# huzjkevin/planar_optical_flow

Measured on AMD Instinct MI355X. Metric: scans/sec, flow-only preprocess of 450-pt synthetic scan pairs, batch 4096 per GPU (+ flow EPE vs reference oracle), higher is better.
Workload: dtype f32 flow arithmetic (float32 outputs) + f64 exact association / mask decisions; the float64-output instantiation (the reference's float64 operation order) is `value_f64`

## Files before the change

planar_optical_flow_amd/csrc/scan_flow.hip:

```cpp
#include <cmath>
#include <cstdlib>
#include <type_traits>

#include "pof_common.h"

namespace {

constexpr int kThreads = 256;

__global__ void laser_phi_kernel(double start, double stop, double step, int n, double *tab)
{
    int i = blockIdx.x * blockDim.x + threadIdx.x;
    if (i >= n) return;
    double p = (double)i * step;
    p = p + start;
    if (i == n - 1 && n > 1) p = stop;
    double s, c;
    sincos(p, &s, &c);
    tab[i] = p;
    tab[n + 2 * i] = c;
    tab[n + 2 * i + 1] = s;
}

struct PreArgs {
// ... 542 lines not shown
                    gx[k] = gy[k] = 0.0f;
                    if (bidx[k] > 0) {
                        double wx, wy;
                        if (ndet[q] <= kInline) {
                            wx = s_det[q][bidx[k] - 1][0];
                            wy = s_det[q][bidx[k] - 1][1];
                            cls[k] = s_lab[q][bidx[k] - 1];
                        } else {
                            const double *w = a.ws_det + (long long)(dfirst + bidx[k] - 1) * kDetStride;
                            wx = w[0];
                            wy = w[1];
                            cls[k] = (long long)w[4];
                        }
                        gx[k] = (float)(wy * cs[k] - wx * sn[k]);
                        gy[k] = (float)((wx * cs[k] + wy * sn[k]) - (double)r[q][k]);
                    }
                }
                if (PTS == 2) {
                    if (a.closest) stream_ll2(reinterpret_cast<long long *>(a.closest), o / 2, bidx[0], bidx[PTS - 1]);
                    if (a.target_cls) stream_ll2(reinterpret_cast<long long *>(a.target_cls), o / 2, cls[0], cls[PTS - 1]);
                    if (a.target_reg) stream_f4(a.target_reg, o / 2, gx[0], gy[0], gx[PTS - 1], gy[PTS - 1]);
                } else {
                    if (a.closest) a.closest[o] = bidx[0];
                    if (a.target_cls) a.target_cls[o] = cls[0];
                    if (a.target_reg) reinterpret_cast<float2 *>(a.target_reg)[o] = make_float2(gx[0], gy[0]);
                }
            }
        }

        if (ok) {
            if (PTS == 2) {
                if (a.dyn_mask) stream_f2(a.dyn_mask, o / 2, dmask[0], dmask[PTS - 1]);
                if (a.valid_mask) stream_f2(a.valid_mask, o / 2, vmask[0], vmask[PTS - 1]);
                if (a.exclude_mask) stream_f2(a.exclude_mask, o / 2, dmask[0] * vmask[0], dmask[PTS - 1] * vmask[PTS - 1]);
            } else {
                if (a.dyn_mask) a.dyn_mask[o] = dmask[0];
                if (a.valid_mask) a.valid_mask[o] = vmask[0];
                if (a.exclude_mask) a.exclude_mask[o] = dmask[0] * vmask[0];
            }
        }
    }
}

constexpr int kMaxSlots = POF_SCAN_MAX_SLOTS;
constexpr int kWaveLds = 2 * kImgBytes;

enum : unsigned {
    kOutXy = 1u << 0, kOutFlow = 1u << 1, kHasDets = 1u << 2, kOutClosest = 1u << 3, kOutCls = 1u << 4,
    kOutReg = 1u << 5, kOutDyn = 1u << 6, kOutValid = 1u << 7, kOutExcl = 1u << 8, kCanonical = 1u << 9,
    kKindShift = 10,
};
constexpr int kCfgHeadline = (int)(kOutFlow | kHasDets | kOutCls | kOutReg | kOutExcl | kCanonical);

struct FlatBatch {
    const float *ranges;
    long long sample_stride;
    void *xy, *flow;
    int64_t *closest, *target_cls;
    float *target_reg, *dyn_mask, *valid_mask, *exclude_mask;
    const int32_t *det_offsets;
    const double *ws_rec, *ws_det;
    int B;
    int wave0;
};
static_assert(sizeof(FlatBatch) % 8 == 0, "FlatBatch is read from the kernel arguments in 8-byte words");

struct FlatArgs {
    const double *tab;
    const float *tabf;
    int N, halfN;
    unsigned magic_m;
    int magic_s;
    unsigned flags;
    int nb;
    int total_waves;
    int main_blocks;
    double ra[3], sd[3], sa[3];
    int lb[3];
    float m_dyn;
    float thr_assoc;
    float m_assoc;
    int uni_waves;
    unsigned uni_m;
    int uni_s;
    int pad_[2];
    int wave0[kMaxSlots];
    FlatBatch b[kMaxSlots];
};

struct ParamsMulti {
    int nb;
    int first, total;
    int uni_blocks;
    unsigned uni_m;
    int uni_s;
    int blk0[kMaxSlots + 1];
    PreArgs p[kMaxSlots];
};

template <typename T>
__device__ __forceinline__ T fma_t(T a, T b, T c);
template <>
__device__ __forceinline__ double fma_t<double>(double a, double b, double c) { return fma(a, b, c); }
template <>
__device__ __forceinline__ float fma_t<float>(float a, float b, float c) { return fmaf(a, b, c); }

template <typename T>
__device__ __forceinline__ void apply_motion_t(int kind, T px, T py, T m0, T m1, T m2, T m3, T t0, T t1, T dph,
                                               T &fx, T &fy)
{
    if (kind == 0) {
        fx = fma_t<T>(py, m1, px * m0) - t0;
        fy = fma_t<T>(py, m3, px * m2) - t1;
    } else if (kind == 1) {
        fx = (fma_t<T>(py, m1, px * m0) - t0) - px;
        fy = (fma_t<T>(py, m3, px * m2) - t1) - py;
    } else if (kind == 2) {
        fx = -t0 - (py * -dph);
        fy = -t1 - (px * dph);
    } else if (kind == 3) {
        fx = ((T)0 - m0 * py + m1) * m3;
        fy = ((m0 * px - (T)0) + m2) * m3;
    } else {
        fx = fma_t<T>(py, m1, px * m0) + t0;
        fy = fma_t<T>(py, m3, px * m2) + t1;
    }
}

template <int CFG>
struct FlatCfg {
    unsigned rt;
    __device__ __forceinline__ bool has(unsigned bit) const { return CFG >= 0 ? ((unsigned)CFG & bit) != 0 : (rt & bit) != 0; }
    __device__ __forceinline__ int kind() const { return CFG >= 0 ? (CFG >> kKindShift) & 7 : (int)(rt >> kKindShift) & 7; }
};

using D2V = double __attribute__((ext_vector_type(2)));

struct RunLoads {
    float2 rv;
    float4 tf;
    D2V t0v, t1v;
    int local, q;
    bool ok;
};

template <typename OutT>
__device__ __forceinline__ RunLoads flat_loads(const FlatArgs &L, const FlatBatch &bt, const int lane, const int sA,
                                               const int l0)
{
    constexpr bool kF32 = sizeof(OutT) == 4;
    RunLoads in;
    int local = l0 + lane;
    const int q = local >= L.halfN ? 1 : 0;
    local -= q ? L.halfN : 0;
    in.local = local;
    in.q = q;
    in.ok = sA + q < bt.B;
    const unsigned i0 = 2u * (unsigned)local;
    const GLOBAL_AS float *rowA = (const GLOBAL_AS float *)bt.ranges + (long long)sA * bt.sample_stride;
    const unsigned roff = (q && in.ok ? (unsigned)bt.sample_stride : 0u) + i0;
    const F2V rr = *(const GLOBAL_AS F2V *)(rowA + roff);
    in.rv = make_float2(rr.x, rr.y);
    in.tf = make_float4(0.f, 0.f, 0.f, 0.f);
    in.t0v = D2V{0.0, 0.0};
    in.t1v = D2V{0.0, 0.0};
    if (kF32 && L.tabf) {
        in.tf = *reinterpret_cast<const float4 *>(L.tabf + 2u * i0);
    } else {
        const double *tab_cs = L.tab + L.N;
        in.t0v = *reinterpret_cast<const D2V *>(tab_cs + 2u * i0);
        in.t1v = *reinterpret_cast<const D2V *>(tab_cs + 2u * i0 + 2);
    }
    return in;
}

template <typename OutT, int CFG>
__device__ __forceinline__ void flat_run(const FlatArgs &L, const FlatBatch &bt, const FlatCfg<CFG> cfg,
                                         const unsigned char *lds, const int lane, const int sA, const int l0,
                                         const long long pair0, const RunLoads &in)
{
    constexpr bool kF32 = sizeof(OutT) == 4;
    const int halfN = L.halfN, N = L.N;
    const int local = in.local, q = in.q;
    const int b = sA + q;
    const bool ok = in.ok;
    const int i0 = 2 * local;
    const float2 rv = in.rv;
    const double *tab_cs = L.tab + N;
    float csf[2], snf[2];
    const D2V t0v = in.t0v, t1v = in.t1v;
    if (kF32 && L.tabf) {
        csf[0] = in.tf.x; snf[0] = in.tf.y; csf[1] = in.tf.z; snf[1] = in.tf.w;
    } else {
        csf[0] = (float)t0v.x; snf[0] = (float)t0v.y; csf[1] = (float)t1v.x; snf[1] = (float)t1v.y;
    }
    const float r[2] = {rv.x, rv.y};
    F2V pxf = {r[0] * csf[0], r[1] * csf[1]}, pyf = {r[0] * snf[0], r[1] * snf[1]};
    auto cs64 = [&](int k) { return tab_cs[2u * (unsigned)(i0 + k)]; };
    auto sn64 = [&](int k) { return tab_cs[2u * (unsigned)(i0 + k) + 1]; };
    auto p64x = [&](int k) { return (double)r[k] * cs64(k); };
    auto p64y = [&](int k) { return (double)r[k] * sn64(k); };
    const unsigned char *hdr = lds + q * kImgBytes;

    if (cfg.has(kOutXy) && ok) {
        OutT *xy = static_cast<OutT *>(bt.xy) + 4 * pair0;
        store2<OutT>(xy, 2u * (unsigned)lane, p64x(0), p64y(0));
        store2<OutT>(xy, 2u * (unsigned)lane + 1, p64x(1), p64y(1));
    }

    if (cfg.has(kOutFlow)) {
        const int kind = cfg.kind();
        if (kF32 && kind != 1) {
            const float4 ma = *reinterpret_cast<const float4 *>(hdr);
            const float4 mb = *reinterpret_cast<const float4 *>(hdr + 16);
            float fxs[2], fys[2];
#pragma unroll
            for (int k = 0; k < 2; ++k) {
                float fx, fy;
                apply_motion_t<float>(kind, pxf[k], pyf[k], ma.x, ma.y, ma.z, ma.w, mb.x, mb.y, mb.z, fx, fy);
                if (cfg.has(kCanonical)) {
                    const float gx = fmaf(csf[k], fx, -snf[k] * fy);
                    const float gy = fmaf(snf[k], fx, csf[k] * fy);
                    fx = gx;
                    fy = gy;
                }
                fxs[k] = fx;
                fys[k] = fy;
            }
            if (ok) stream_f4(reinterpret_cast<float *>(bt.flow) + 4 * pair0, (unsigned)lane, fxs[0], fys[0], fxs[1], fys[1]);
        } else {
            const double *mot = reinterpret_cast<const double *>(hdr + kImgMot);
            const double m0 = mot[0], m1 = mot[1], m2 = mot[2], m3 = mot[3];
            const double tr0 = mot[4], tr1 = mot[5], dph = mot[6];
            OutT *fl = static_cast<OutT *>(bt.flow) + 4 * pair0;
            double cs[2], sn[2];
            if (kF32 && L.tabf) {
                cs[0] = cs64(0); sn[0] = sn64(0); cs[1] = cs64(1); sn[1] = sn64(1);
            } else {
                cs[0] = t0v.x; sn[0] = t0v.y; cs[1] = t1v.x; sn[1] = t1v.y;
            }
            double f[4];
#pragma unroll
            for (int k = 0; k < 2; ++k) {
                double fx, fy;
                apply_motion(kind, (double)r[k] * cs[k], (double)r[k] * sn[k], m0, m1, m2, m3, tr0, tr1, dph, fx, fy);
                if (cfg.has(kCanonical)) {
                    const double gx = cs[k] * fx + (-sn[k]) * fy;
                    const double gy = sn[k] * fx + cs[k] * fy;
                    fx = gx;
                    fy = gy;
                }
                f[2 * k] = fx;
                f[2 * k + 1] = fy;
            }
            if (ok) {
                if (kF32) {
                    stream_f4(reinterpret_cast<float *>(fl), (unsigned)lane, (float)f[0], (float)f[1], (float)f[2], (float)f[3]);
                } else {
                    D2V v0 = {f[0], f[1]}, v1 = {f[2], f[3]};
                    GLOBAL_AS D2V *dst = (GLOBAL_AS D2V *)fl + 2u * (unsigned)lane;
                    __builtin_nontemporal_store(v0, dst);
                    __builtin_nontemporal_store(v1, dst + 1);
                }
            }
        }
    }

    float vmask[2], dmask[2];
#pragma unroll
    for (int k = 0; k < 2; ++k) {
        vmask[k] = (r[k] >= 20.0f) ? 0.0f : 1.0f;
        dmask[k] = 1.0f;
    }

    if (cfg.has(kHasDets)) {
        const bool want_assoc = cfg.has(kOutClosest) || cfg.has(kOutCls) || cfg.has(kOutReg);
        const bool want_dyn = cfg.has(kOutDyn) || cfg.has(kOutExcl);
        const int4 h1 = *reinterpret_cast<const int4 *>(hdr + 16);
        const int2 h2 = *reinterpret_cast<const int2 *>(hdr + 32);
        const int2 h3 = *reinterpret_cast<const int2 *>(hdr + 40);
        const int nd = ok ? h1.w : 0;
        const int n_in = min(nd, kInline);
        const int nA = l0 < halfN ? reinterpret_cast<const int *>(lds)[7] : 0;
        const int nB = l0 + 63 >= halfN ? reinterpret_cast<const int *>(lds + kImgBytes)[7] : 0;
        const int n_loop = __builtin_amdgcn_readfirstlane(min(max(nA, nB), kInline));
        F2V mind = {INFINITY, INFINITY};
        const unsigned char *ent = hdr + kImgScreen;
        for (int j = 0; j < n_loop; ++j) {
            const float4 e = *reinterpret_cast<const float4 *>(ent + 16 * j);
            const F2V cx2 = {e.x, e.x}, cy2 = {e.y, e.y}, ns2 = {e.z, e.z};
            const F2V ex = pxf - cx2, ey = pyf - cy2;
            F2V d = __builtin_elementwise_fma(ey, ey, ns2);
            d = __builtin_elementwise_fma(ex, ex, d);
            mind = __builtin_elementwise_min(mind, d);
        }
        const bool samp_far = (h3.x | h3.y) != 0;
        int bidx[2] = {0, 0};
        int dfirst = 0;
        auto cls_of = [&](int j) { return ((j < 4 ? h2.x : h2.y) >> (8 * (j & 3))) & 3; };
        auto sel3 = [&](const double *v, int c) { return c == 0 ? v[0] : (c == 1 ? v[1] : v[2]); };
        auto candidate = [&](int k, int j1, double s2, double ra) {
            if (bidx[k] != 0) {
                double wx, wy, wra;
                if (bidx[k] <= kInline) {
                    const D2V c = *reinterpret_cast<const D2V *>(hdr + kImgCtr + 16 * (bidx[k] - 1));
                    wx = c.x; wy = c.y; wra = sel3(L.ra, cls_of(bidx[k] - 1));
                } else {
                    const GLOBAL_AS double *w = (const GLOBAL_AS double *)bt.ws_det + (long long)(dfirst + bidx[k] - 1) * kDetStride;
                    wx = w[0]; wy = w[1]; wra = w[2];
                }
                const double exd = p64x(k) - wx, eyd = p64y(k) - wy;
                if (!(sqrt(s2) - ra < sqrt(exd * exd + eyd * eyd) - wra)) return;
            }
            bidx[k] = j1;
        };
#pragma unroll
        for (int k = 0; k < 2; ++k) {
            const bool exk = samp_far || !(fabsf(pxf[k]) + fabsf(pyf[k]) < 100.0f);
            bool need_dyn = false;
            if (!exk && mind[k] <= -L.m_dyn) dmask[k] = 0.0f;
            else need_dyn = want_dyn && (exk || mind[k] <= L.m_dyn);
            bool need_assoc = want_assoc && (exk || mind[k] <= L.thr_assoc);
            if (need_assoc && !exk) {
                int ncand = 0, jc = 0;
                bool unsure = false;
                for (int j = 0; j < n_in; ++j) {
                    const float4 e = *reinterpret_cast<const float4 *>(ent + 16 * j);
                    const float exf = pxf[k] - e.x, eyf = pyf[k] - e.y;
                    const float d = fmaf(exf, exf, fmaf(eyf, eyf, e.z));
                    if (d <= e.w + L.m_assoc) {
                        if (d <= e.w - L.m_assoc) { ++ncand; jc = j; }
                        else unsure = true;
                    }
                }
                if (!unsure && ncand <= 1) {
                    if (ncand == 1) bidx[k] = jc + 1;
                    need_assoc = false;
                }
            }
            if (need_dyn || need_assoc) {
                const double pxd = p64x(k), pyd = p64y(k);
                for (int j = 0; j < n_in; ++j) {
                    const D2V c = *reinterpret_cast<const D2V *>(hdr + kImgCtr + 16 * j);
                    const int cl = cls_of(j);
                    const double exd = pxd - c.x, eyd = pyd - c.y;
                    const double s2 = exd * exd + eyd * eyd;
                    if (need_dyn && s2 <= sel3(L.sd, cl)) dmask[k] = 0.0f;
                    if (need_assoc && s2 <= sel3(L.sa, cl)) candidate(k, j + 1, s2, sel3(L.ra, cl));
                }
            }
        }
        if (nd > kInline) {
            dfirst = ((const GLOBAL_AS int32_t *)bt.det_offsets)[b];
            for (int j = kInline; j < nd; ++j) {
                const GLOBAL_AS double *w = (const GLOBAL_AS double *)bt.ws_det + (long long)(dfirst + j) * kDetStride;
                const double cx = w[0], cy = w[1], ra = w[2], sd = w[3], sa = w[5];
#pragma unroll
                for (int k = 0; k < 2; ++k) {
                    const double exd = p64x(k) - cx, eyd = p64y(k) - cy;
                    const double s2 = exd * exd + eyd * eyd;
                    if (s2 <= sd) dmask[k] = 0.0f;
                    if (want_assoc && s2 <= sa) candidate(k, j + 1, s2, ra);
                }
            }
        }
        if (ok && want_assoc) {
            long long cls[2];
            float gx[2], gy[2];
#pragma unroll
            for (int k = 0; k < 2; ++k) {
                cls[k] = 0;
                gx[k] = gy[k] = 0.0f;
                if (bidx[k] > 0) {
                    double wx, wy;
                    if (bidx[k] <= kInline) {
                        const D2V c = *reinterpret_cast<const D2V *>(hdr + kImgCtr + 16 * (bidx[k] - 1));
                        wx = c.x; wy = c.y;
                        const int cl = cls_of(bidx[k] - 1);
                        cls[k] = cl == 0 ? L.lb[0] : (cl == 1 ? L.lb[1] : L.lb[2]);
                    } else {
                        const GLOBAL_AS double *w = (const GLOBAL_AS double *)bt.ws_det + (long long)(dfirst + bidx[k] - 1) * kDetStride;
                        wx = w[0];
                        wy = w[1];
                        cls[k] = (long long)w[4];
                    }
                    const double c = cs64(k), sn_ = sn64(k);
                    gx[k] = (float)(wy * c - wx * sn_);
                    gy[k] = (float)((wx * c + wy * sn_) - (double)r[k]);
                }
            }
            if (cfg.has(kOutClosest)) stream_ll2(reinterpret_cast<long long *>(bt.closest) + 2 * pair0, (unsigned)lane, bidx[0], bidx[1]);
            if (cfg.has(kOutCls)) stream_ll2(reinterpret_cast<long long *>(bt.target_cls) + 2 * pair0, (unsigned)lane, cls[0], cls[1]);
            if (cfg.has(kOutReg)) stream_f4(bt.target_reg + 4 * pair0, (unsigned)lane, gx[0], gy[0], gx[1], gy[1]);
        }
    }

    if (ok) {
        if (cfg.has(kOutDyn)) stream_f2(bt.dyn_mask + 2 * pair0, (unsigned)lane, dmask[0], dmask[1]);
        if (cfg.has(kOutValid)) stream_f2(bt.valid_mask + 2 * pair0, (unsigned)lane, vmask[0], vmask[1]);
        if (cfg.has(kOutExcl)) stream_f2(bt.exclude_mask + 2 * pair0, (unsigned)lane, dmask[0] * vmask[0], dmask[1] * vmask[1]);
    }
}

typedef const __attribute__((address_space(4))) unsigned char *kernarg_ptr;
template <typename S>
__device__ __forceinline__ S kernarg_struct(kernarg_ptr p)
{
    static_assert(sizeof(S) % 8 == 0, "kernarg slots are read in 8-byte words");
    S out;
    unsigned long long *w = reinterpret_cast<unsigned long long *>(&out);
#pragma unroll
    for (int i = 0; i < (int)(sizeof(S) / 8); ++i)
        w[i] = *reinterpret_cast<const __attribute__((address_space(4))) unsigned long long *>(p + 8 * i);
    return out;
}
constexpr size_t kFlatArgsKernargBytes = (sizeof(FlatArgs) + 7) & ~(size_t)7;

template <typename OutT, int CFG, int THREADS, int CPW>
__global__ __launch_bounds__(THREADS, 8) void scan_flat_kernel(const FlatArgs L, const ParamsMulti P)
{
    constexpr int WAVES = THREADS / 64;
    __shared__ __align__(16) unsigned char smem[WAVES][kWaveLds];
    kernarg_ptr ka = (kernarg_ptr)__builtin_amdgcn_kernarg_segment_ptr();
    int sblock = (int)blockIdx.x;
    if (sblock >= P.first) {
        if (sblock < P.first + P.total) {
#ifndef POF_FLAT_NO_PARAMS
            const int blk = sblock - P.first;
            int k = 0, b0 = P.blk0[0];
            if (P.uni_blocks) {
                k = (int)(__umulhi((unsigned)blk, P.uni_m) >> P.uni_s);
                b0 = k * P.uni_blocks;
            } else {
#pragma unroll
                for (int i = 1; i < kMaxSlots; ++i) k += (blk >= P.blk0[i]) ? 1 : 0;
                k = __builtin_amdgcn_readfirstlane(k);
#pragma unroll
                for (int i = 1; i < kMaxSlots; ++i) b0 = (k >= i) ? P.blk0[i] : b0;
            }
            const auto *pa = reinterpret_cast<const __attribute__((address_space(4))) PreArgs *>(
                ka + kFlatArgsKernargBytes + offsetof(ParamsMulti, p) + (size_t)k * sizeof(PreArgs));
            params_work<false, false>(pa, (blk - b0) * THREADS + (int)threadIdx.x);
#endif
            return;
        }
        sblock -= P.total;
    }
    const int wv = __builtin_amdgcn_readfirstlane((int)threadIdx.x >> 6);
    const int lane = (int)threadIdx.x & 63;
    const int w = sblock * WAVES + wv;
    if (w >= L.total_waves) return;
    int k = 0;
    if (L.uni_waves) {
        k = (int)(__umulhi((unsigned)w, L.uni_m) >> L.uni_s);
    } else {
#pragma unroll
        for (int i = 1; i < kMaxSlots; ++i) k += (w >= L.wave0[i]) ? 1 : 0;
    }
    k = __builtin_amdgcn_readfirstlane(k);
    const FlatBatch bt = kernarg_struct<FlatBatch>(ka + offsetof(FlatArgs, b) + (size_t)k * sizeof(FlatBatch));
    const FlatCfg<CFG> cfg{L.flags};
    unsigned char *lds = smem[wv];

    const unsigned p0 = (unsigned)(w - bt.wave0) * (64u * CPW);
    const int sA = (int)(__umulhi(p0, L.magic_m) >> L.magic_s);
    const int l0 = (int)(p0 - (unsigned)sA * (unsigned)L.halfN);

    RunLoads in[CPW];
#pragma unroll
    for (int c = 0; c < CPW; ++c) in[c] = flat_loads<OutT>(L, bt, lane, sA, l0 + 64 * c);

    if (cfg.has(kOutFlow) || cfg.has(kHasDets)) {
        {
            const int sq = lane >> 5, i = lane & 31;
            if (i < kImgBytes / 16) {
                const double *rec = bt.ws_rec + (long long)min(sA + sq, bt.B - 1) * kRecStride;
                *reinterpret_cast<F4V *>(lds + sq * kImgBytes + 16 * i) = ((const GLOBAL_AS F4V *)(rec + kRecImg))[i];
            }
        }
        __builtin_amdgcn_fence(__ATOMIC_RELEASE, "wavefront");
        __builtin_amdgcn_wave_barrier();
        __builtin_amdgcn_fence(__ATOMIC_ACQUIRE, "wavefront");
    }
#pragma unroll
    for (int c = 0; c < CPW; ++c)
        flat_run<OutT, CFG>(L, bt, cfg, lds, lane, sA, l0 + 64 * c, (long long)p0 + 64 * c, in[c]);
}

template <typename T>
__global__ void rotate_flow_kernel(const T *in, T *out, const double *tab, long long total, int N,
                                   int to_canonical)
{
    long long p = (long long)blockIdx.x * blockDim.x + threadIdx.x;
    if (p >= total) return;
    int i = (int)(p % N);
    T gx, gy;
    pof_rotate_flow_point<T>(tab[N + 2 * i], tab[N + 2 * i + 1], in[2 * p], in[2 * p + 1], to_canonical, gx, gy);
    out[2 * p] = gx;
    out[2 * p + 1] = gy;
}

__global__ void det_to_canonical_kernel(const float *ranges, const double *tab, const double *det_r,
                                        const double *det_phi, double *dx, double *dy, long long total,
                                        int N)
{
    long long p = (long long)blockIdx.x * blockDim.x + threadIdx.x;
    if (p >= total) return;
    int i = (int)(p % N);
    double s, c;
    sincos(det_phi[p] - tab[i], &s, &c);
    dx[p] = s * det_r[p];
    dy[p] = c * det_r[p] - (double)ranges[p];
}

__global__ void canonical_to_det_kernel(const float *ranges, const double *tab, const double *dx,
                                        const double *dy, double *det_r, double *det_phi,
                                        long long total, int N)
{
    long long p = (long long)blockIdx.x * blockDim.x + threadIdx.x;
    if (p >= total) return;
    int i = (int)(p % N);
    double ty = (double)ranges[p] + dy[p];
    double tphi = atan2(dx[p], ty);
    det_phi[p] = tphi + tab[i];
    det_r[p] = ty / cos(tphi);
}

template <typename OutT, int PTS, int SPB>
__global__ __launch_bounds__(kThreads, 8) void scan_preprocess_kernel(PreArgs a)
{
    scan_main<OutT, PTS, SPB>(a, blockIdx.y);
}

template <typename OutT, int PTS, int SPB>
__global__ __launch_bounds__(kThreads, 8) void scan_preprocess_chain_kernel(PreArgs a, PreArgs nx, int main_rows)
{
    if ((int)blockIdx.y >= main_rows) {
        if (blockIdx.x == 0) params_work<false, true>(&nx, ((int)blockIdx.y - main_rows) * kThreads + threadIdx.x);
        return;
// ... 183 lines not shown
}

template <typename OutT, int CFG>
void flat_dispatch(int threads, int cpw, dim3 grid, hipStream_t s, const FlatArgs &L, const ParamsMulti &P)
{
#define POF_FLAT_CASE(T, C) \
    if (threads == T && cpw == C) { scan_flat_kernel<OutT, CFG, T, C><<<grid, T, 0, s>>>(L, P); return; }
    POF_FLAT_CASE(64, 1)
    POF_FLAT_CASE(64, 2)
    POF_FLAT_CASE(128, 1)
    POF_FLAT_CASE(128, 2)
    POF_FLAT_CASE(256, 1)
    POF_FLAT_CASE(256, 2)
#undef POF_FLAT_CASE
}

int bind_next(const pof_scan_inputs *next, PreArgs &nx, int *jobs)
{
    *jobs = 0;
    if (next->B < 0 || next->D < 0 || next->B > 65535) return POF_E_BADARG;
    if (next->want_flow && (!next->odom0 || !next->odom1)) return POF_E_BADARG;
    if (next->flow_kind < 0 || next->flow_kind > 4) return POF_E_BADARG;
    if (next->det_offsets && next->D > 0 && (!next->det_rphi || !next->det_cls)) return POF_E_BADARG;
    if (next->B > 0 && (next->want_flow || next->det_offsets)) {
        if (!next->workspace ||
            next->workspace_bytes < pof_scan_preprocess_workspace_bytes(next->B, next->det_offsets ? next->D : 0))
            return POF_E_WORKSPACE;
        nx.B = next->B; nx.D = next->det_offsets ? next->D : 0;
        nx.odom0 = next->odom0; nx.odom1 = next->odom1; nx.flow_kind = next->flow_kind;
        nx.flow = next->want_flow ? reinterpret_cast<void *>(1) : nullptr;
        nx.det_offsets = next->det_offsets; nx.det_rphi = next->det_rphi; nx.det_cls = next->det_cls;
        fill_class_constants(nx, next->det_offsets != nullptr, next->assoc_radius, next->labels, next->dyn_radius);
        bind_workspace(nx, next->workspace, next->B);
        *jobs = params_job_count(nx.B, nx.det_offsets != nullptr);
    }
    return POF_OK;
}

void magic_u31(unsigned d, unsigned *m, int *sh)
{
    int lg = 1;
    while ((1u << lg) < d) ++lg;
    *m = (unsigned)(((1ull << (31 + lg)) + d - 1) / d);
    *sh = lg - 1;
}

int launch_flat(const FlatBatch *cur, int n_cur, const FlatCommon &c, const pof_scan_inputs *const *next, int n_next,
                hipStream_t s)
{
    int threads, cpw, ppos;
    flat_tuning(&threads, &cpw, &ppos);
    if (!flat_shape_ok(c.N, cpw)) cpw = 1;
    FlatArgs L = {};
    L.tab = c.tab; L.tabf = c.tabf; L.N = c.N; L.halfN = c.N / 2;
    int lg = 0;
    while ((1u << lg) < (unsigned)L.halfN) ++lg;
    L.magic_m = (unsigned)(((1ull << (31 + lg)) + (unsigned)L.halfN - 1) / (unsigned)L.halfN);
    L.magic_s = lg - 1;
    L.flags = flat_flags(cur[0], c);
    L.nb = n_cur;
    PreArgs cc = {};
    fill_class_constants(cc, cur[0].det_offsets != nullptr, c.assoc_radius, c.labels, c.dyn_radius);
    L.ra[0] = cc.ra0; L.ra[1] = cc.ra1; L.ra[2] = cc.ra2;
    L.sd[0] = cc.sd0; L.sd[1] = cc.sd1; L.sd[2] = cc.sd2;
    L.sa[0] = cc.sa0; L.sa[1] = cc.sa1; L.sa[2] = cc.sa2;
    L.lb[0] = cc.lb0; L.lb[1] = cc.lb1; L.lb[2] = cc.lb2;
    double md = 0.0, ma = 0.0, gap = -HUGE_VAL, span = 0.0;
    for (int k = 0; k < 3; ++k) {
        md = std::fmax(md, 1e-3 + 1e-4 * std::fmax(L.sd[k], 0.0));
        ma = std::fmax(ma, 1e-3 + 1e-4 * std::fmax(std::fmax(L.sd[k], L.sa[k]), 0.0));
        gap = std::fmax(gap, L.sa[k] - L.sd[k]);
        span = std::fmax(span, std::fabs(L.sa[k] - L.sd[k]));
    }
    L.m_dyn = f32_round_up(md * (1.0 + 1e-6));
    L.m_assoc = f32_round_up(ma * 1.001 + 2.4e-7 * span);
    L.thr_assoc = f32_round_up(gap + (double)L.m_assoc + 1e-6 * std::fabs(gap));
    long long waves = 0;
    const long long pairs_per_wave = 64LL * cpw;
    for (int i = 0; i < n_cur; ++i) {
        if (flat_flags(cur[i], c) != L.flags) return POF_E_BADARG;
        L.b[i] = cur[i];
        L.b[i].wave0 = (int)waves;
        L.wave0[i] = (int)waves;
        waves += ((long long)cur[i].B * L.halfN + pairs_per_wave - 1) / pairs_per_wave;
        if ((long long)cur[i].B * L.halfN >= (1LL << 31) || waves >= (1LL << 30)) return POF_E_SHAPE;
    }
    for (int i = n_cur; i < kMaxSlots; ++i) L.wave0[i] = 0x7fffffff;
    L.total_waves = (int)waves;
    L.uni_waves = 0; L.uni_m = 0; L.uni_s = 0;
    if (n_cur > 0 && waves % n_cur == 0) {
        const long long per = waves / n_cur;
        bool same = per > 1;
        for (int i = 0; i < n_cur && same; ++i) same = L.wave0[i] == (int)(per * i);
        if (same) { L.uni_waves = (int)per; magic_u31((unsigned)per, &L.uni_m, &L.uni_s); }
    }
    const int wpb = threads / 64;
    L.main_blocks = (int)((waves + wpb - 1) / wpb);
    ParamsMulti P = {};
    P.nb = 0;
    int extra = 0;
    for (int i = 0; i < n_next; ++i) {
        PreArgs nx = {};
        int jobs = 0;
        const int rc = bind_next(next[i], nx, &jobs);
        if (rc != POF_OK) return rc;
        if (jobs == 0) continue;
        P.blk0[P.nb] = extra;
        P.p[P.nb] = nx;
        extra += (jobs + threads - 1) / threads;
        ++P.nb;
    }
    for (int i = P.nb; i <= kMaxSlots; ++i) P.blk0[i] = extra;
    P.total = extra;
    P.uni_blocks = 0; P.uni_m = 0; P.uni_s = 0;
    if (P.nb > 0 && extra % P.nb == 0) {
        const int per = extra / P.nb;
        bool same = per > 1;
        for (int i = 0; i < P.nb && same; ++i) same = P.blk0[i] == per * i;
        if (same) { P.uni_blocks = per; magic_u31((unsigned)per, &P.uni_m, &P.uni_s); }
    }
    P.first = (int)((long long)L.main_blocks * ppos / 100);
    if (L.main_blocks + extra == 0) return POF_OK;
    dim3 grid((unsigned)(L.main_blocks + extra));
    const bool headline = (L.flags == (unsigned)kCfgHeadline);
    if (c.out_f64) {
        if (headline) flat_dispatch<double, kCfgHeadline>(threads, cpw, grid, s, L, P);
        else flat_dispatch<double, -1>(threads, cpw, grid, s, L, P);
    } else {
        if (headline) flat_dispatch<float, kCfgHeadline>(threads, cpw, grid, s, L, P);
        else flat_dispatch<float, -1>(threads, cpw, grid, s, L, P);
    }
    return POF_OK;
}

int launch_preprocess(const float *ranges, long long sample_stride, int B, int N, const double *tab,
                      const double *odom0, const double *odom1, int flow_kind, int canonical, int out_f64,
                      void *xy, void *flow, const int32_t *det_offsets, const double *det_rphi,
                      const uint8_t *det_cls, int D, const double *assoc_radius, const int32_t *labels,
                      const double *dyn_radius, int64_t *closest, int64_t *target_cls, float *target_reg,
                      float *dyn_mask, float *valid_mask, float *exclude_mask, void *workspace,
                      size_t workspace_bytes, int phases, const pof_scan_inputs *next, pof_stream_t stream)
{
    if ((phases & 3) == 0 || (phases & ~3)) return POF_E_BADARG;
    if (!ranges || !tab || B < 0 || N < 1 || D < 0) return POF_E_BADARG;
    if (flow && (!odom0 || !odom1)) return POF_E_BADARG;
    if (flow_kind < 0 || flow_kind > 4) return POF_E_BADARG;
    if (det_offsets && (!assoc_radius || !labels || !dyn_radius)) return POF_E_BADARG;
    if (det_offsets && D > 0 && (!det_rphi || !det_cls)) return POF_E_BADARG;
    if (sample_stride < N) return POF_E_SHAPE;
    if (B == 0) return POF_OK;
    if (B > 65535) return POF_E_SHAPE;
    const bool need_ws = flow || det_offsets;
    if (need_ws && (!workspace || workspace_bytes < pof_scan_preprocess_workspace_bytes(B, det_offsets ? D : 0)))
        return POF_E_WORKSPACE;
    PreArgs a;
    a.ranges = ranges; a.sample_stride = sample_stride; a.B = B; a.N = N; a.D = det_offsets ? D : 0;
    a.tab = tab;
    a.odom0 = odom0; a.odom1 = odom1; a.flow_kind = flow_kind; a.canonical = canonical;
    a.xy = xy; a.flow = flow; a.det_offsets = det_offsets; a.det_rphi = det_rphi; a.det_cls = det_cls;
    fill_class_constants(a, det_offsets != nullptr, assoc_radius, labels, dyn_radius);
    a.closest = closest; a.target_cls = target_cls; a.target_reg = target_reg;
    a.dyn_mask = dyn_mask; a.valid_mask = valid_mask; a.exclude_mask = exclude_mask;
    bind_workspace(a, workspace, B);
    hipStream_t s = pof_stream(stream);
    if (need_ws && (phases & 1)) {
        const int total = params_job_count(B, det_offsets != nullptr);
        scan_params_kernel<<<(total + 255) / 256, 256, 0, s>>>(a);
        POF_CHECK_LAUNCH();
    }
    if (!(phases & 2)) return POF_OK;

    PreArgs nx = a;
    int next_jobs = 0;
    if (next) {
// ... 225 lines not shown
```

Baseline: 395.6 million.

## Repack kernel args into hot 64-byte blocks and park trig table in LDS

Reorders the flat-kernel argument structs so the per-launch and per-slot hot fields each fit one 64-byte block, loaded with a single wide scalar kernarg load, while rarely used fields are read lazily through kernarg pointers. The double cos/sin table entries are staged into per-wave LDS instead of being re-read from global memory or held in registers across the run. The detection screening loop is also unrolled by four, and mask flags become a bitmask. The aim is to cut scalar load count and register pressure in exchange for more LDS per block and reliance on the new struct layout.

Measured after the change: 404.3 million (median of 3 runs). +2.2%, better.

```diff
diff --git a/planar_optical_flow_amd/csrc/scan_flow.hip b/planar_optical_flow_amd/csrc/scan_flow.hip
--- a/planar_optical_flow_amd/csrc/scan_flow.hip
+++ b/planar_optical_flow_amd/csrc/scan_flow.hip
@@ -618,45 +618,72 @@
 };
 constexpr int kCfgHeadline = (int)(kOutFlow | kHasDets | kOutCls | kOutReg | kOutExcl | kCanonical);
 
+struct FlatBatchHot {
+    const float *ranges;
+    long long sample_stride;
+    const double *ws_rec;
+    int B;
+    int wave0;
+    void *flow;
+    int64_t *target_cls;
+    float *target_reg, *exclude_mask;
+};
 struct FlatBatch {
     const float *ranges;
     long long sample_stride;
-    void *xy, *flow;
-    int64_t *closest, *target_cls;
-    float *target_reg, *dyn_mask, *valid_mask, *exclude_mask;
-    const int32_t *det_offsets;
-    const double *ws_rec, *ws_det;
+    const double *ws_rec;
     int B;
     int wave0;
+    void *flow;
+    int64_t *target_cls;
+    float *target_reg, *exclude_mask;
+    void *xy;
+    int64_t *closest;
+    float *dyn_mask, *valid_mask;
+    const int32_t *det_offsets;
+    const double *ws_det;
+    long long pad_[2];
 };
-static_assert(sizeof(FlatBatch) % 8 == 0, "FlatBatch is read from the kernel arguments in 8-byte words");
-
-struct FlatArgs {
-    const double *tab;
+static_assert(sizeof(FlatBatchHot) == 64 && sizeof(FlatBatch) == 128 && offsetof(FlatBatch, xy) == 64 &&
+              offsetof(FlatBatch, exclude_mask) == offsetof(FlatBatchHot, exclude_mask) &&
+              offsetof(FlatBatch, wave0) == offsetof(FlatBatchHot, wave0), "a slot is two 64-byte blocks");
+
+struct FlatHead {
     const float *tabf;
-    int N, halfN;
+    const double *tab_cs;
+    int p_first, p_total;
+    int total_waves;
+    int uni_waves;
+    unsigned uni_m;
+    int uni_s;
+    int halfN;
     unsigned magic_m;
     int magic_s;
-    unsigned flags;
-    int nb;
-    int total_waves;
-    int main_blocks;
-    double ra[3], sd[3], sa[3];
-    int lb[3];
     float m_dyn;
     float thr_assoc;
     float m_assoc;
-    int uni_waves;
-    unsigned uni_m;
-    int uni_s;
-    int pad_[2];
+};
+static_assert(sizeof(FlatHead) == 64, "the hot words are one 64-byte block");
+
+struct FlatRare {
+    double ra[3], sd[3], sa[3];
+    int lb[3];
+    int pad_;
+};
+
+struct FlatArgs {
+    FlatHead h;
+    unsigned flags;
     int wave0[kMaxSlots];
+    int pad_[7];
     FlatBatch b[kMaxSlots];
+    FlatRare rare;
+    int nb;
+    int main_blocks;
 };
 
 struct ParamsMulti {
     int nb;
-    int first, total;
     int uni_blocks;
     unsigned uni_m;
     int uni_s;
@@ -693,6 +720,26 @@
     }
 }
 
+typedef const __attribute__((address_space(4))) unsigned char *kernarg_ptr;
+using U16V = unsigned __attribute__((ext_vector_type(16)));
+typedef U16V U16V_a4 __attribute__((aligned(4)));
+template <typename S>
+__device__ __forceinline__ S kernarg_hot64(kernarg_ptr p)
+{
+    static_assert(sizeof(S) == 64, "one 64-byte block");
+    S out;
+    U16V v = *reinterpret_cast<const __attribute__((address_space(4))) U16V_a4 *>(p);
+    asm volatile("" : "+s"(v));
+    __builtin_memcpy(&out, &v, 64);
+    return out;
+}
+template <typename S>
+__device__ __forceinline__ const __attribute__((address_space(4))) S *kernarg_lazy(kernarg_ptr p)
+{
+    asm("" : "+s"(p));
+    return reinterpret_cast<const __attribute__((address_space(4))) S *>(p);
+}
+
 template <int CFG>
 struct FlatCfg {
     unsigned rt;
@@ -710,11 +757,16 @@
     bool ok;
 };
 
+#ifdef POF_FLAT_TAB_GLOBAL
+constexpr int kRunTabBytes = 0;
+#else
+constexpr int kRunTabBytes = 2 * 64 * 16;
+#endif
+
 template <typename OutT>
-__device__ __forceinline__ RunLoads flat_loads(const FlatArgs &L, const FlatBatch &bt, const int lane, const int sA,
+__device__ __forceinline__ RunLoads flat_loads(const FlatHead &L, const FlatBatchHot &bt, const int lane, const int sA,
                                                const int l0)
 {
-    constexpr bool kF32 = sizeof(OutT) == 4;
     RunLoads in;
     int local = l0 + lane;
     const int q = local >= L.halfN ? 1 : 0;
@@ -730,46 +782,61 @@
     in.tf = make_float4(0.f, 0.f, 0.f, 0.f);
     in.t0v = D2V{0.0, 0.0};
     in.t1v = D2V{0.0, 0.0};
-    if (kF32 && L.tabf) {
+#ifdef POF_FLAT_TAB_GLOBAL
+    if (sizeof(OutT) == 4 && L.tabf) {
         in.tf = *reinterpret_cast<const float4 *>(L.tabf + 2u * i0);
-    } else {
-        const double *tab_cs = L.tab + L.N;
-        in.t0v = *reinterpret_cast<const D2V *>(tab_cs + 2u * i0);
-        in.t1v = *reinterpret_cast<const D2V *>(tab_cs + 2u * i0 + 2);
-    }
+        return in;
+    }
+#endif
+    const GLOBAL_AS double *tab_cs = (const GLOBAL_AS double *)L.tab_cs;
+    in.t0v = *reinterpret_cast<const GLOBAL_AS D2V *>(tab_cs + 2u * i0);
+    in.t1v = *reinterpret_cast<const GLOBAL_AS D2V *>(tab_cs + 2u * i0 + 2);
     return in;
 }
 
+template <typename OutT>
+__device__ __forceinline__ void flat_park(const FlatHead &L, RunLoads &in, unsigned char *tabl, const int lane)
+{
+#ifdef POF_FLAT_TAB_GLOBAL
+    if (sizeof(OutT) == 4 && L.tabf) return;
+#else
+    *reinterpret_cast<D2V *>(tabl + 16 * lane) = in.t0v;
+    *reinterpret_cast<D2V *>(tabl + 1024 + 16 * lane) = in.t1v;
+#endif
+    in.tf = make_float4((float)in.t0v.x, (float)in.t0v.y, (float)in.t1v.x, (float)in.t1v.y);
+}
+
 template <typename OutT, int CFG>
-__device__ __forceinline__ void flat_run(const FlatArgs &L, const FlatBatch &bt, const FlatCfg<CFG> cfg,
-                                         const unsigned char *lds, const int lane, const int sA, const int l0,
-                                         const long long pair0, const RunLoads &in)
+__device__ __forceinline__ void flat_run(const FlatHead &L, kernarg_ptr ka, const FlatBatchHot &bt, kernarg_ptr slot_p, const FlatCfg<CFG> cfg,
+                                         const unsigned char *lds, const unsigned char *tabl, const int lane,
+                                         const int sA, const int l0, const long long pair0, const RunLoads &in)
 {
     constexpr bool kF32 = sizeof(OutT) == 4;
-    const int halfN = L.halfN, N = L.N;
-    const int local = in.local, q = in.q;
+    const int halfN = L.halfN;
+    const int q = in.q;
     const int b = sA + q;
     const bool ok = in.ok;
-    const int i0 = 2 * local;
     const float2 rv = in.rv;
-    const double *tab_cs = L.tab + N;
-    float csf[2], snf[2];
-    const D2V t0v = in.t0v, t1v = in.t1v;
-    if (kF32 && L.tabf) {
-        csf[0] = in.tf.x; snf[0] = in.tf.y; csf[1] = in.tf.z; snf[1] = in.tf.w;
-    } else {
-        csf[0] = (float)t0v.x; snf[0] = (float)t0v.y; csf[1] = (float)t1v.x; snf[1] = (float)t1v.y;
-    }
+    const float csf[2] = {in.tf.x, in.tf.z}, snf[2] = {in.tf.y, in.tf.w};
     const float r[2] = {rv.x, rv.y};
     F2V pxf = {r[0] * csf[0], r[1] * csf[1]}, pyf = {r[0] * snf[0], r[1] * snf[1]};
-    auto cs64 = [&](int k) { return tab_cs[2u * (unsigned)(i0 + k)]; };
-    auto sn64 = [&](int k) { return tab_cs[2u * (unsigned)(i0 + k) + 1]; };
+#ifdef POF_FLAT_TAB_GLOBAL
+    const double *tab_cs = L.tab_cs;
+    const int i0 = 2 * in.local;
+    auto csn64 = [&](int k) { return D2V{tab_cs[2u * (unsigned)(i0 + k)], tab_cs[2u * (unsigned)(i0 + k) + 1]}; };
+#else
+    auto csn64 = [&](int k) { return *reinterpret_cast<const D2V *>(tabl + 1024 * k + 16 * lane); };
+#endif
+    auto cs64 = [&](int k) { return csn64(k).x; };
+    auto sn64 = [&](int k) { return csn64(k).y; };
     auto p64x = [&](int k) { return (double)r[k] * cs64(k); };
     auto p64y = [&](int k) { return (double)r[k] * sn64(k); };
     const unsigned char *hdr = lds + q * kImgBytes;
+    const auto *rare = kernarg_lazy<FlatRare>(ka + offsetof(FlatArgs, rare));
+    const auto *slot = kernarg_lazy<FlatBatch>(slot_p);
 
     if (cfg.has(kOutXy) && ok) {
-        OutT *xy = static_cast<OutT *>(bt.xy) + 4 * pair0;
+        OutT *xy = static_cast<OutT *>(slot->xy) + 4 * pair0;
         store2<OutT>(xy, 2u * (unsigned)lane, p64x(0), p64y(0));
         store2<OutT>(xy, 2u * (unsigned)lane + 1, p64x(1), p64y(1));
     }
@@ -799,12 +866,13 @@
             const double m0 = mot[0], m1 = mot[1], m2 = mot[2], m3 = mot[3];
             const double tr0 = mot[4], tr1 = mot[5], dph = mot[6];
             OutT *fl = static_cast<OutT *>(bt.flow) + 4 * pair0;
-            double cs[2], sn[2];
-            if (kF32 && L.tabf) {
-                cs[0] = cs64(0); sn[0] = sn64(0); cs[1] = cs64(1); sn[1] = sn64(1);
-            } else {
-                cs[0] = t0v.x; sn[0] = t0v.y; cs[1] = t1v.x; sn[1] = t1v.y;
-            }
+#ifdef POF_FLAT_TAB_GLOBAL
+            const bool held = !(kF32 && L.tabf);
+            const D2V c0 = held ? in.t0v : csn64(0), c1 = held ? in.t1v : csn64(1);
+#else
+            const D2V c0 = csn64(0), c1 = csn64(1);
+#endif
+            const double cs[2] = {c0.x, c1.x}, sn[2] = {c0.y, c1.y};
             double f[4];
 #pragma unroll
             for (int k = 0; k < 2; ++k) {
@@ -832,12 +900,7 @@
         }
     }
 
-    float vmask[2], dmask[2];
-#pragma unroll
-    for (int k = 0; k < 2; ++k) {
-        vmask[k] = (r[k] >= 20.0f) ? 0.0f : 1.0f;
-        dmask[k] = 1.0f;
-    }
+    unsigned dhit = 0;
 
     if (cfg.has(kHasDets)) {
         const bool want_assoc = cfg.has(kOutClosest) || cfg.has(kOutCls) || cfg.has(kOutReg);
@@ -852,27 +915,38 @@
         const int n_loop = __builtin_amdgcn_readfirstlane(min(max(nA, nB), kInline));
         F2V mind = {INFINITY, INFINITY};
         const unsigned char *ent = hdr + kImgScreen;
-        for (int j = 0; j < n_loop; ++j) {
-            const float4 e = *reinterpret_cast<const float4 *>(ent + 16 * j);
-            const F2V cx2 = {e.x, e.x}, cy2 = {e.y, e.y}, ns2 = {e.z, e.z};
-            const F2V ex = pxf - cx2, ey = pyf - cy2;
-            F2V d = __builtin_elementwise_fma(ey, ey, ns2);
-            d = __builtin_elementwise_fma(ex, ex, d);
-            mind = __builtin_elementwise_min(mind, d);
+        static_assert(kInline % 4 == 0, "the screen is read four entries at a time");
+#pragma unroll 1
+        for (int j = 0; j < n_loop; j += 4) {
+            float4 e[4];
+#pragma unroll
+            for (int u = 0; u < 4; ++u) e[u] = *reinterpret_cast<const float4 *>(ent + 16 * (j + u));
+#pragma unroll
+            for (int u = 0; u < 4; ++u) {
+                const F2V cx2 = {e[u].x, e[u].x}, cy2 = {e[u].y, e[u].y}, ns2 = {e[u].z, e[u].z};
+                const F2V ex = pxf - cx2, ey = pyf - cy2;
+                F2V d = __builtin_elementwise_fma(ey, ey, ns2);
+                d = __builtin_elementwise_fma(ex, ex, d);
+                mind = __builtin_elementwise_min(mind, d);
+            }
         }
         const bool samp_far = (h3.x | h3.y) != 0;
         int bidx[2] = {0, 0};
         int dfirst = 0;
         auto cls_of = [&](int j) { return ((j < 4 ? h2.x : h2.y) >> (8 * (j & 3))) & 3; };
-        auto sel3 = [&](const double *v, int c) { return c == 0 ? v[0] : (c == 1 ? v[1] : v[2]); };
+        auto sel3 = [&](const __attribute__((address_space(4))) double *v, int c) {
+            double v0 = v[0], v1 = v[1], v2 = v[2];
+            asm("" : "+s"(v0), "+s"(v1), "+s"(v2));
+            return c == 0 ? v0 : (c == 1 ? v1 : v2);
+        };
         auto candidate = [&](int k, int j1, double s2, double ra) {
             if (bidx[k] != 0) {
                 double wx, wy, wra;
                 if (bidx[k] <= kInline) {
                     const D2V c = *reinterpret_cast<const D2V *>(hdr + kImgCtr + 16 * (bidx[k] - 1));
-                    wx = c.x; wy = c.y; wra = sel3(L.ra, cls_of(bidx[k] - 1));
+                    wx = c.x; wy = c.y; wra = sel3(rare->ra, cls_of(bidx[k] - 1));
                 } else {
-                    const GLOBAL_AS double *w = (const GLOBAL_AS double *)bt.ws_det + (long long)(dfirst + bidx[k] - 1) * kDetStride;
+                    const GLOBAL_AS double *w = (const GLOBAL_AS double *)slot->ws_det + (long long)(dfirst + bidx[k] - 1) * kDetStride;
                     wx = w[0]; wy = w[1]; wra = w[2];
                 }
                 const double exd = p64x(k) - wx, eyd = p64y(k) - wy;
@@ -884,7 +958,7 @@
         for (int k = 0; k < 2; ++k) {
             const bool exk = samp_far || !(fabsf(pxf[k]) + fabsf(pyf[k]) < 100.0f);
             bool need_dyn = false;
-            if (!exk && mind[k] <= -L.m_dyn) dmask[k] = 0.0f;
+            if (!exk && mind[k] <= -L.m_dyn) dhit |= 1u << k;
             else need_dyn = want_dyn && (exk || mind[k] <= L.m_dyn);
             bool need_assoc = want_assoc && (exk || mind[k] <= L.thr_assoc);
             if (need_assoc && !exk) {
@@ -911,27 +985,27 @@
                     const int cl = cls_of(j);
                     const double exd = pxd - c.x, eyd = pyd - c.y;
                     const double s2 = exd * exd + eyd * eyd;
-                    if (need_dyn && s2 <= sel3(L.sd, cl)) dmask[k] = 0.0f;
-                    if (need_assoc && s2 <= sel3(L.sa, cl)) candidate(k, j + 1, s2, sel3(L.ra, cl));
+                    if (need_dyn && s2 <= sel3(rare->sd, cl)) dhit |= 1u << k;
+                    if (need_assoc && s2 <= sel3(rare->sa, cl)) candidate(k, j + 1, s2, sel3(rare->ra, cl));
                 }
             }
         }
         if (nd > kInline) {
-            dfirst = ((const GLOBAL_AS int32_t *)bt.det_offsets)[b];
+            dfirst = ((const GLOBAL_AS int32_t *)slot->det_offsets)[b];
             for (int j = kInline; j < nd; ++j) {
-                const GLOBAL_AS double *w = (const GLOBAL_AS double *)bt.ws_det + (long long)(dfirst + j) * kDetStride;
+                const GLOBAL_AS double *w = (const GLOBAL_AS double *)slot->ws_det + (long long)(dfirst + j) * kDetStride;
                 const double cx = w[0], cy = w[1], ra = w[2], sd = w[3], sa = w[5];
 #pragma unroll
                 for (int k = 0; k < 2; ++k) {
                     const double exd = p64x(k) - cx, eyd = p64y(k) - cy;
                     const double s2 = exd * exd + eyd * eyd;
-                    if (s2 <= sd) dmask[k] = 0.0f;
+                    if (s2 <= sd) dhit |= 1u << k;
                     if (want_assoc && s2 <= sa) candidate(k, j + 1, s2, ra);
                 }
             }
         }
         if (ok && want_assoc) {
-            long long cls[2];
+            int cls[2];
             float gx[2], gy[2];
 #pragma unroll
             for (int k = 0; k < 2; ++k) {
@@ -943,56 +1017,51 @@
                         const D2V c = *reinterpret_cast<const D2V *>(hdr + kImgCtr + 16 * (bidx[k] - 1));
                         wx = c.x; wy = c.y;
                         const int cl = cls_of(bidx[k] - 1);
-                        cls[k] = cl == 0 ? L.lb[0] : (cl == 1 ? L.lb[1] : L.lb[2]);
+                        int l0_ = rare->lb[0], l1_ = rare->lb[1], l2_ = rare->lb[2];
+                        asm("" : "+s"(l0_), "+s"(l1_), "+s"(l2_));
+                        cls[k] = cl == 0 ? l0_ : (cl == 1 ? l1_ : l2_);
                     } else {
-                        const GLOBAL_AS double *w = (const GLOBAL_AS double *)bt.ws_det + (long long)(dfirst + bidx[k] - 1) * kDetStride;
+                        const GLOBAL_AS double *w = (const GLOBAL_AS double *)slot->ws_det + (long long)(dfirst + bidx[k] - 1) * kDetStride;
                         wx = w[0];
                         wy = w[1];
-                        cls[k] = (long long)w[4];
+                        cls[k] = (int)w[4];
                     }
                     const double c = cs64(k), sn_ = sn64(k);
                     gx[k] = (float)(wy * c - wx * sn_);
                     gy[k] = (float)((wx * c + wy * sn_) - (double)r[k]);
                 }
             }
-            if (cfg.has(kOutClosest)) stream_ll2(reinterpret_cast<long long *>(bt.closest) + 2 * pair0, (unsigned)lane, bidx[0], bidx[1]);
+            if (cfg.has(kOutClosest)) stream_ll2(reinterpret_cast<long long *>(slot->closest) + 2 * pair0, (unsigned)lane, bidx[0], bidx[1]);
             if (cfg.has(kOutCls)) stream_ll2(reinterpret_cast<long long *>(bt.target_cls) + 2 * pair0, (unsigned)lane, cls[0], cls[1]);
             if (cfg.has(kOutReg)) stream_f4(bt.target_reg + 4 * pair0, (unsigned)lane, gx[0], gy[0], gx[1], gy[1]);
         }
     }
 
     if (ok) {
-        if (cfg.has(kOutDyn)) stream_f2(bt.dyn_mask + 2 * pair0, (unsigned)lane, dmask[0], dmask[1]);
-        if (cfg.has(kOutValid)) stream_f2(bt.valid_mask + 2 * pair0, (unsigned)lane, vmask[0], vmask[1]);
+        const float dmask[2] = {(dhit & 1u) ? 0.0f : 1.0f, (dhit & 2u) ? 0.0f : 1.0f};
+        const float vmask[2] = {(r[0] >= 20.0f) ? 0.0f : 1.0f, (r[1] >= 20.0f) ? 0.0f : 1.0f};
+        if (cfg.has(kOutDyn)) stream_f2(slot->dyn_mask + 2 * pair0, (unsigned)lane, dmask[0], dmask[1]);
+        if (cfg.has(kOutValid)) stream_f2(slot->valid_mask + 2 * pair0, (unsigned)lane, vmask[0], vmask[1]);
         if (cfg.has(kOutExcl)) stream_f2(bt.exclude_mask + 2 * pair0, (unsigned)lane, dmask[0] * vmask[0], dmask[1] * vmask[1]);
     }
 }
 
-typedef const __attribute__((address_space(4))) unsigned char *kernarg_ptr;
-template <typename S>
-__device__ __forceinline__ S kernarg_struct(kernarg_ptr p)
-{
-    static_assert(sizeof(S) % 8 == 0, "kernarg slots are read in 8-byte words");
-    S out;
-    unsigned long long *w = reinterpret_cast<unsigned long long *>(&out);
-#pragma unroll
-    for (int i = 0; i < (int)(sizeof(S) / 8); ++i)
-        w[i] = *reinterpret_cast<const __attribute__((address_space(4))) unsigned long long *>(p + 8 * i);
-    return out;
-}
 constexpr size_t kFlatArgsKernargBytes = (sizeof(FlatArgs) + 7) & ~(size_t)7;
 
 template <typename OutT, int CFG, int THREADS, int CPW>
 __global__ __launch_bounds__(THREADS, 8) void scan_flat_kernel(const FlatArgs L, const ParamsMulti P)
 {
     constexpr int WAVES = THREADS / 64;
-    __shared__ __align__(16) unsigned char smem[WAVES][kWaveLds];
+    constexpr int kLds = kWaveLds + CPW * kRunTabBytes;
+    __shared__ __align__(16) unsigned char smem[WAVES][kLds];
     kernarg_ptr ka = (kernarg_ptr)__builtin_amdgcn_kernarg_segment_ptr();
+    const FlatCfg<CFG> cfg{CFG < 0 ? *reinterpret_cast<const __attribute__((address_space(4))) unsigned *>(ka + offsetof(FlatArgs, flags)) : 0u};
+    const FlatHead H = kernarg_hot64<FlatHead>(ka + offsetof(FlatArgs, h));
     int sblock = (int)blockIdx.x;
-    if (sblock >= P.first) {
-        if (sblock < P.first + P.total) {
+    if (sblock >= H.p_first) {
+        if (sblock < H.p_first + H.p_total) {
 #ifndef POF_FLAT_NO_PARAMS
-            const int blk = sblock - P.first;
+            const int blk = sblock - H.p_first;
             int k = 0, b0 = P.blk0[0];
             if (P.uni_blocks) {
                 k = (int)(__umulhi((unsigned)blk, P.uni_m) >> P.uni_s);
@@ -1010,47 +1079,50 @@
 #endif
             return;
         }
-        sblock -= P.total;
+        sblock -= H.p_total;
     }
     const int wv = __builtin_amdgcn_readfirstlane((int)threadIdx.x >> 6);
     const int lane = (int)threadIdx.x & 63;
     const int w = sblock * WAVES + wv;
-    if (w >= L.total_waves) return;
+    if (w >= H.total_waves) return;
     int k = 0;
-    if (L.uni_waves) {
-        k = (int)(__umulhi((unsigned)w, L.uni_m) >> L.uni_s);
+    if (H.uni_waves) {
+        k = (int)(__umulhi((unsigned)w, H.uni_m) >> H.uni_s);
     } else {
-#pragma unroll
-        for (int i = 1; i < kMaxSlots; ++i) k += (w >= L.wave0[i]) ? 1 : 0;
+        const auto *wave0 = kernarg_lazy<int>(ka + offsetof(FlatArgs, wave0));
+#pragma unroll
+        for (int i = 1; i < kMaxSlots; ++i) k += (w >= wave0[i]) ? 1 : 0;
     }
     k = __builtin_amdgcn_readfirstlane(k);
-    const FlatBatch bt = kernarg_struct<FlatBatch>(ka + offsetof(FlatArgs, b) + (size_t)k * sizeof(FlatBatch));
-    const FlatCfg<CFG> cfg{L.flags};
+    kernarg_ptr slot_p = ka + offsetof(FlatArgs, b) + (size_t)k * sizeof(FlatBatch);
+    const FlatBatchHot bt = kernarg_hot64<FlatBatchHot>(slot_p);
     unsigned char *lds = smem[wv];
 
     const unsigned p0 = (unsigned)(w - bt.wave0) * (64u * CPW);
-    const int sA = (int)(__umulhi(p0, L.magic_m) >> L.magic_s);
-    const int l0 = (int)(p0 - (unsigned)sA * (unsigned)L.halfN);
+    const int sA = (int)(__umulhi(p0, H.magic_m) >> H.magic_s);
+    const int l0 = (int)(p0 - (unsigned)sA * (unsigned)H.halfN);
 
     RunLoads in[CPW];
 #pragma unroll
-    for (int c = 0; c < CPW; ++c) in[c] = flat_loads<OutT>(L, bt, lane, sA, l0 + 64 * c);
-
-    if (cfg.has(kOutFlow) || cfg.has(kHasDets)) {
+    for (int c = 0; c < CPW; ++c) in[c] = flat_loads<OutT>(H, bt, lane, sA, l0 + 64 * c);
+
+    {
         {
             const int sq = lane >> 5, i = lane & 31;
-            if (i < kImgBytes / 16) {
+            if ((cfg.has(kOutFlow) || cfg.has(kHasDets)) && i < kImgBytes / 16) {
                 const double *rec = bt.ws_rec + (long long)min(sA + sq, bt.B - 1) * kRecStride;
                 *reinterpret_cast<F4V *>(lds + sq * kImgBytes + 16 * i) = ((const GLOBAL_AS F4V *)(rec + kRecImg))[i];
             }
         }
+#pragma unroll
+        for (int c = 0; c < CPW; ++c) flat_park<OutT>(H, in[c], lds + kWaveLds + c * kRunTabBytes, lane);
         __builtin_amdgcn_fence(__ATOMIC_RELEASE, "wavefront");
         __builtin_amdgcn_wave_barrier();
         __builtin_amdgcn_fence(__ATOMIC_ACQUIRE, "wavefront");
     }
 #pragma unroll
     for (int c = 0; c < CPW; ++c)
-        flat_run<OutT, CFG>(L, bt, cfg, lds, lane, sA, l0 + 64 * c, (long long)p0 + 64 * c, in[c]);
+        flat_run<OutT, CFG>(H, ka, bt, slot_p, cfg, lds, lds + kWaveLds + c * kRunTabBytes, lane, sA, l0 + 64 * c, (long long)p0 + 64 * c, in[c]);
 }
 
 template <typename T>
@@ -1340,29 +1412,31 @@
     flat_tuning(&threads, &cpw, &ppos);
     if (!flat_shape_ok(c.N, cpw)) cpw = 1;
     FlatArgs L = {};
-    L.tab = c.tab; L.tabf = c.tabf; L.N = c.N; L.halfN = c.N / 2;
+    FlatHead &H = L.h;
+    FlatRare &R = L.rare;
+    H.tab_cs = c.tab + c.N; H.tabf = c.tabf; H.halfN = c.N / 2;
     int lg = 0;
-    while ((1u << lg) < (unsigned)L.halfN) ++lg;
-    L.magic_m = (unsigned)(((1ull << (31 + lg)) + (unsigned)L.halfN - 1) / (unsigned)L.halfN);
-    L.magic_s = lg - 1;
+    while ((1u << lg) < (unsigned)H.halfN) ++lg;
+    H.magic_m = (unsigned)(((1ull << (31 + lg)) + (unsigned)H.halfN - 1) / (unsigned)H.halfN);
+    H.magic_s = lg - 1;
     L.flags = flat_flags(cur[0], c);
     L.nb = n_cur;
     PreArgs cc = {};
     fill_class_constants(cc, cur[0].det_offsets != nullptr, c.assoc_radius, c.labels, c.dyn_radius);
-    L.ra[0] = cc.ra0; L.ra[1] = cc.ra1; L.ra[2] = cc.ra2;
-    L.sd[0] = cc.sd0; L.sd[1] = cc.sd1; L.sd[2] = cc.sd2;
-    L.sa[0] = cc.sa0; L.sa[1] = cc.sa1; L.sa[2] = cc.sa2;
-    L.lb[0] = cc.lb0; L.lb[1] = cc.lb1; L.lb[2] = cc.lb2;
+    R.ra[0] = cc.ra0; R.ra[1] = cc.ra1; R.ra[2] = cc.ra2;
+    R.sd[0] = cc.sd0; R.sd[1] = cc.sd1; R.sd[2] = cc.sd2;
+    R.sa[0] = cc.sa0; R.sa[1] = cc.sa1; R.sa[2] = cc.sa2;
+    R.lb[0] = cc.lb0; R.lb[1] = cc.lb1; R.lb[2] = cc.lb2;
     double md = 0.0, ma = 0.0, gap = -HUGE_VAL, span = 0.0;
     for (int k = 0; k < 3; ++k) {
-        md = std::fmax(md, 1e-3 + 1e-4 * std::fmax(L.sd[k], 0.0));
-        ma = std::fmax(ma, 1e-3 + 1e-4 * std::fmax(std::fmax(L.sd[k], L.sa[k]), 0.0));
-        gap = std::fmax(gap, L.sa[k] - L.sd[k]);
-        span = std::fmax(span, std::fabs(L.sa[k] - L.sd[k]));
-    }
-    L.m_dyn = f32_round_up(md * (1.0 + 1e-6));
-    L.m_assoc = f32_round_up(ma * 1.001 + 2.4e-7 * span);
-    L.thr_assoc = f32_round_up(gap + (double)L.m_assoc + 1e-6 * std::fabs(gap));
+        md = std::fmax(md, 1e-3 + 1e-4 * std::fmax(R.sd[k], 0.0));
+        ma = std::fmax(ma, 1e-3 + 1e-4 * std::fmax(std::fmax(R.sd[k], R.sa[k]), 0.0));
+        gap = std::fmax(gap, R.sa[k] - R.sd[k]);
+        span = std::fmax(span, std::fabs(R.sa[k] - R.sd[k]));
+    }
+    H.m_dyn = f32_round_up(md * (1.0 + 1e-6));
+    H.m_assoc = f32_round_up(ma * 1.001 + 2.4e-7 * span);
+    H.thr_assoc = f32_round_up(gap + (double)H.m_assoc + 1e-6 * std::fabs(gap));
     long long waves = 0;
     const long long pairs_per_wave = 64LL * cpw;
     for (int i = 0; i < n_cur; ++i) {
@@ -1370,17 +1444,17 @@
         L.b[i] = cur[i];
         L.b[i].wave0 = (int)waves;
         L.wave0[i] = (int)waves;
-        waves += ((long long)cur[i].B * L.halfN + pairs_per_wave - 1) / pairs_per_wave;
-        if ((long long)cur[i].B * L.halfN >= (1LL << 31) || waves >= (1LL << 30)) return POF_E_SHAPE;
+        waves += ((long long)cur[i].B * H.halfN + pairs_per_wave - 1) / pairs_per_wave;
+        if ((long long)cur[i].B * H.halfN >= (1LL << 31) || waves >= (1LL << 30)) return POF_E_SHAPE;
     }
     for (int i = n_cur; i < kMaxSlots; ++i) L.wave0[i] = 0x7fffffff;
-    L.total_waves = (int)waves;
-    L.uni_waves = 0; L.uni_m = 0; L.uni_s = 0;
+    H.total_waves = (int)waves;
+    H.uni_waves = 0; H.uni_m = 0; H.uni_s = 0;
     if (n_cur > 0 && waves % n_cur == 0) {
         const long long per = waves / n_cur;
         bool same = per > 1;
         for (int i = 0; i < n_cur && same; ++i) same = L.wave0[i] == (int)(per * i);
-        if (same) { L.uni_waves = (int)per; magic_u31((unsigned)per, &L.uni_m, &L.uni_s); }
+        if (same) { H.uni_waves = (int)per; magic_u31((unsigned)per, &H.uni_m, &H.uni_s); }
     }
     const int wpb = threads / 64;
     L.main_blocks = (int)((waves + wpb - 1) / wpb);
@@ -1399,7 +1473,7 @@
         ++P.nb;
     }
     for (int i = P.nb; i <= kMaxSlots; ++i) P.blk0[i] = extra;
-    P.total = extra;
+    H.p_total = extra;
     P.uni_blocks = 0; P.uni_m = 0; P.uni_s = 0;
     if (P.nb > 0 && extra % P.nb == 0) {
         const int per = extra / P.nb;
@@ -1407,7 +1481,7 @@
         for (int i = 0; i < P.nb && same; ++i) same = P.blk0[i] == per * i;
         if (same) { P.uni_blocks = per; magic_u31((unsigned)per, &P.uni_m, &P.uni_s); }
     }
-    P.first = (int)((long long)L.main_blocks * ppos / 100);
+    H.p_first = (int)((long long)L.main_blocks * ppos / 100);
     if (L.main_blocks + extra == 0) return POF_OK;
     dim3 grid((unsigned)(L.main_blocks + extra));
     const bool headline = (L.flags == (unsigned)kCfgHeadline);
```
